# vshiv18/khoice

Measured on AMD Instinct MI355X. Metric: distinct k-mers/sec (k=31, canonical), higher is better.
Workload: dtype u64

## Files before the change

khoice_amd/csrc/kh_engine.cpp:

```cpp
#include <hip/hip_runtime.h>

#include <algorithm>
#include <atomic>
#include <thread>
#include <chrono>
#include <cmath>
#include <memory>
#include <cstdarg>
#include <cstdio>
#include <cstdlib>
#include <cstring>
#include <map>
#include <mutex>
#include <string>
#include <vector>

#include "../../include/khoice_hip.h"
#include "kh_engine.h"
#include "kh_launch.h"
#include "kh_skm_rec.h"

static thread_local std::string g_last_error;

int kh_fail(int code, const char* fmt, ...) {
// ... 1602 lines not shown
    static constexpr u32 spill_cap = 1u << 20, big_cap = 16384u;
#ifdef KH_STAMPS
    Tmp d_stamps;
#endif
    explicit SkmStage(kh_ctx* c) : pin{c} {}
};
static int skm_prepare(kh_ctx* c, int nseq, const uint8_t* const* seqs, const uint64_t* lens, int on_device,
                       const int* group_of, int ngroups, int k, bool by_group, u32 force_slots, u32 fan_hint, SkmStage* s) {
    TagLayout* L = &s->L;
    if (!skm_form_k(k)) return KH_OK;
    if ((!by_group && nseq > KH_TAG_MAX_OPS) || ngroups > KH_TAG_MAX_OPS) return KH_OK;
    KHCHK(tag_layout(L, nseq, group_of, ngroups, by_group));
    if (L->nbins > (u32)KH_TAG_MAX_BINS) return KH_OK;
    const u64 positions = kmer_positions(nseq, lens, k, &s->bases);
    if (!skm_plan(k, positions, std::max(L->fan, fan_hint), force_slots, c->cus, &s->g)) return KH_OK;
    const SkmGeometry& g = s->g;
    const size_t rec_bytes = g.two ? 32 : 16;
    const size_t reg1_bytes = rec_bytes * (size_t)g.nb1 * g.cap1, reg2_bytes = rec_bytes * (size_t)g.nslots * g.cap2;
    HIPCHK(hipSetDevice(c->dev));
    {
        size_t free_b = 0, total_b = 0;
        if (hipMemGetInfo(&free_b, &total_b) == hipSuccess &&
            reg1_bytes + reg2_bytes + s->bases + (64u << 20) > free_b + c->pool.cached_bytes)
            return KH_OK;
    }
    hipStream_t st = c->st;

    u32 tile_pos = KH_TILE;
    {
        const u64 want_tiles = 8ull * (u64)std::max(1, c->cus);
        while (tile_pos > (u32)KH_SUBTILE && (positions + tile_pos - 1) / tile_pos < want_tiles) tile_pos >>= 1;
    }
    std::vector<KhSeg> segs(nseq);
    std::vector<u64> pack_off(nseq);
    std::vector<KhTile> tiles;
    u64 seq_bytes = 0;
    for (int i = 0; i < nseq; ++i) {
        KhSeg& sg = segs[i];
        memset(&sg, 0, sizeof sg);
        const u64 len = lens[L->perm[i]];
        pack_off[i] = seq_bytes;
        sg.len = len;
        sg.npos = len >= (u64)k ? len - k + 1 : 0;
        sg.ntiles = (u32)((sg.npos + tile_pos - 1) / tile_pos);
        sg.tile_base = (u32)tiles.size();
        for (u32 t = 0; t < sg.ntiles; ++t) tiles.push_back(KhTile{(u32)i, t});
        seq_bytes += (len + 15) & ~15ull;
    }
    seq_bytes += 256;
    const u32 ntiles = (u32)tiles.size();
    const u32 reps = g.ugrid;
    const size_t hist_words = (size_t)reps * L->nbins;
    const size_t off_ctl = 8 * hist_words, off_inst = off_ctl + 32, off_dup = off_inst + 8 * (size_t)nseq,
                 off_cur1 = off_dup + 8 * 64, off_cur2 = off_cur1 + 4 * (size_t)KH_SKM_CUR1_STRIDE * g.nb1,
                 off_ginfo = off_cur2 + 4 * (size_t)((g.nslots + 3) & ~3u), off_tags = off_ginfo + 256,
                 off_segs = off_tags + (((size_t)nseq + 15) & ~(size_t)15), off_tiles = off_segs + sizeof(KhSeg) * nseq,
                 ws_bytes = off_tiles + sizeof(KhTile) * (size_t)std::max<u32>(1, ntiles);
    const u32 spill_cap = SkmStage::spill_cap;
    bool need_pack = false;
    for (int i = 0; i < nseq; ++i)
        if (!(on_device && (reinterpret_cast<uintptr_t>(seqs[L->perm[i]]) & 15) == 0)) need_pack = true;
    TMP_ALLOC(s->d_seq, c, need_pack ? seq_bytes : 256);
    TMP_ALLOC(s->d_ws, c, ws_bytes);
    TMP_ALLOC(s->d_reg1, c, reg1_bytes);
    TMP_ALLOC(s->d_reg2, c, reg2_bytes);
    TMP_ALLOC(s->d_spill, c, (size_t)spill_cap * (rec_bytes + 4) + (size_t)SkmStage::big_cap * 4);
    const size_t up_bytes = ws_bytes - off_ginfo;
    const size_t down_bytes = off_cur1;
    PIN_ALLOC(s->pin, up_bytes + down_bytes + 64);
    u8* h_up = static_cast<u8*>(s->pin.p);
    s->h_down = h_up + ((up_bytes + 63) & ~(size_t)63);
    c->prof_begin(KC_COPY_IN);
    for (int i = 0; i < nseq; ++i) {
        const uint8_t* src = seqs[L->perm[i]];
        if (on_device && (reinterpret_cast<uintptr_t>(src) & 15) == 0) { segs[i].seq = src; continue; }
        segs[i].seq = s->d_seq.as<u8>() + pack_off[i];
        if (!segs[i].len) continue;
        HIPCHK(hipMemcpyAsync(s->d_seq.as<u8>() + pack_off[i], src, segs[i].len,
                              on_device ? hipMemcpyDeviceToDevice : hipMemcpyHostToDevice, st));
        c->stat.text_packed += segs[i].len;
    }
    memcpy(h_up + (off_segs - off_ginfo), segs.data(), sizeof(KhSeg) * nseq);
    if (ntiles) memcpy(h_up + (off_tiles - off_ginfo), tiles.data(), sizeof(KhTile) * (size_t)ntiles);
    L->words(reinterpret_cast<u32*>(h_up), h_up + (off_tags - off_ginfo), group_of);
    u8* wsp = s->d_ws.as<u8>();
    HIPCHK(hipMemsetAsync(wsp, 0, off_ginfo, st));
    HIPCHK(hipMemcpyAsync(wsp + off_ginfo, h_up, up_bytes, hipMemcpyHostToDevice, st));
    c->prof_end();

    KhSkmJob& job = s->job;
    job.seg_tag = by_group ? wsp + off_tags : nullptr;
    job.segs = reinterpret_cast<const KhSeg*>(wsp + off_segs);
    job.tiles = reinterpret_cast<const KhTile*>(wsp + off_tiles);
    job.reg1 = s->d_reg1.as<uint4>();
    job.reg2 = s->d_reg2.as<uint4>();
    job.cur1 = reinterpret_cast<u32*>(wsp + off_cur1);
    job.cur2 = reinterpret_cast<u32*>(wsp + off_cur2);
    job.inst = reinterpret_cast<unsigned long long*>(wsp + off_inst);
    job.dup = reinterpret_cast<unsigned long long*>(wsp + off_dup);
    job.ginfo = reinterpret_cast<const u32*>(wsp + off_ginfo);
    job.hist = reinterpret_cast<unsigned long long*>(wsp);
    job.ctl = reinterpret_cast<u32*>(wsp + off_ctl);
    job.tile_pos = tile_pos;
    job.k = k; job.m = g.m; job.w = g.w; job.nmax = g.nmax;
    job.nslots = g.nslots; job.S = g.S; job.nb1 = g.nb1; job.cap1 = g.cap1; job.cap2 = g.cap2;
    job.nbins = L->nbins; job.abase = L->abase; job.reps = reps; job.nops = by_group ? (u32)ngroups : (u32)nseq;
    job.spill_rec = s->d_spill.as<uint4>();
    job.spill_slot = reinterpret_cast<u32*>(s->d_spill.as<u8>() + (size_t)spill_cap * rec_bytes);
    job.big_list = reinterpret_cast<u32*>(s->d_spill.as<u8>() + (size_t)spill_cap * (rec_bytes + 4));
    job.spill_cap = spill_cap;
    job.big_cap = SkmStage::big_cap;
    s->ntiles = ntiles;
#ifdef KH_STAMPS
    const u64 nst = std::max<u64>(ntiles, g.nslots);
    TMP_ALLOC(s->d_stamps, c, 128 * nst);
    HIPCHK(hipMemsetAsync(s->d_stamps.b->p, 0, 128 * nst, st));
    kh_debug_set_stamps_skm(s->d_stamps.as<u64>());
#endif
    c->prof_begin(KC_SKM_SCATTER);
    if (g.two) kh_launch_skm2_scatter(job, ntiles, st);
    else kh_launch_skm_scatter(job, ntiles, st);
    c->prof_end();
#ifdef KH_STAMPS
    report_stamps(c, "skm_scatter (second sub-tile: codes / hashes / minima / slots+count / - / append / barrier / -)", s->d_stamps.b, ntiles);
    HIPCHK(hipMemsetAsync(s->d_stamps.b->p, 0, 128 * nst, st));
    kh_debug_set_stamps_skm(nullptr);
#endif
    c->prof_begin(KC_SKM_REGROUP);
    if (g.two) kh_launch_skm2_regroup(job, st);
    else kh_launch_skm_regroup(job, st);
    c->prof_end();
#ifdef KH_STAMPS
    kh_debug_set_stamps_skm(s->d_stamps.as<u64>());
#endif
    s->staged = true;
    return KH_OK;
}
static int exp1_skm(kh_ctx* c, const Exp1In& in, uint64_t* within_hist, uint64_t* across_hist, uint64_t* distinct_per_seq,
                    bool* done, bool by_group = false) {
    *done = false;
    SkmStage s(c);
    KHCHK(skm_prepare(c, in.nseq, in.seqs, in.lens, in.on_device, in.group_of, in.ngroups, in.k, by_group, 0, 0, &s));
    if (!s.staged) return KH_OK;
    const TagLayout& L = s.L;
    const SkmGeometry& g = s.g;
    const KhSkmJob& job = s.job;
    hipStream_t st = c->st;
    c->prof_begin(KC_SKM_UNION);
    if (g.two) kh_launch_skm2_union(job, in.cs, g.ugrid, st);
    else kh_launch_skm_union(job, in.cs, g.ugrid, st);
    c->prof_end();
    HIPCHK(hipGetLastError());
#ifdef KH_STAMPS
    report_stamps(c, "skm_union (scan barrier / owner / expand / insert / barrier / read-out / barrier / flush)", s.d_stamps.b, g.nslots);
    kh_debug_set_stamps_skm(nullptr);
#endif
    if (getenv("KHOICE_SKM_DEBUG")) {
        std::vector<u32> h1(g.nb1), h2(g.nslots);
        HIPCHK(hipMemcpy2DAsync(h1.data(), 4, job.cur1, 4 * (size_t)KH_SKM_CUR1_STRIDE, 4, g.nb1, hipMemcpyDeviceToHost, st));
        HIPCHK(hipMemcpyAsync(h2.data(), job.cur2, 4 * (size_t)g.nslots, hipMemcpyDeviceToHost, st));
        u32 hc[8];
        HIPCHK(hipMemcpyAsync(hc, job.ctl, 32, hipMemcpyDeviceToHost, st));
        HIPCHK(hipStreamSynchronize(st));
        u64 t1 = 0, t2 = 0;
        u32 m1 = 0, m2 = 0;
        for (u32 v : h1) { t1 += v; m1 = std::max(m1, v); }
        for (u32 v : h2) { t2 += v; m2 = std::max(m2, v); }
        fprintf(stderr, "[skm] k=%d m=%d w=%u nmax=%u positions=%llu records=%llu (%.2f k-mers each) nb1=%u S=%u nslots=%u | "
                        "coarse: mean %.0f max %u cap %u | slot: mean %.1f max %u cap %u | tiles %u x %u | expanded: %u k-mers | errors %u spilled %u overfull slots %u\n",
                in.k, g.m, g.w, g.nmax, (unsigned long long)g.positions, (unsigned long long)t1, (double)g.positions / std::max<u64>(1, t1),
                g.nb1, g.S, g.nslots, (double)t1 / g.nb1, m1, g.cap1, (double)t2 / g.nslots, m2, g.cap2, s.ntiles, job.tile_pos, hc[3], hc[0], hc[5], hc[6]);
    }
    u8* h_down = s.h_down;
    u8* wsp = s.d_ws.as<u8>();
    auto down = [&](const void* d) { return h_down + (static_cast<const u8*>(d) - wsp); };
    const size_t down_bytes = down(job.cur1) - h_down;
    HIPCHK(hipMemcpyAsync(h_down, wsp, down_bytes, hipMemcpyDeviceToHost, st));
    HIPCHK(hipStreamSynchronize(st));
    const u64* h_hist = reinterpret_cast<const u64*>(h_down);
    const u32* h_ctl = reinterpret_cast<const u32*>(down(job.ctl));
    if (h_ctl[6] && !(h_ctl[0] & (KH_ERR_CAPACITY | KH_ERR_ORDER))) {
        if (h_ctl[5] > SkmStage::spill_cap || h_ctl[6] > SkmStage::big_cap) { c->stat.retries++; return KH_OK; }
        c->stat.big_slots += h_ctl[6];
        c->prof_begin(KC_SKM_BIG);
        if (g.two) kh_launch_skm2_big(job, in.cs, h_ctl[6], st);
        else kh_launch_skm_big(job, in.cs, h_ctl[6], st);
        c->prof_end();
        HIPCHK(hipGetLastError());
        HIPCHK(hipMemcpyAsync(h_down, wsp, down_bytes, hipMemcpyDeviceToHost, st));
        HIPCHK(hipStreamSynchronize(st));
    }
    const u64* h_inst = reinterpret_cast<const u64*>(down(job.inst));
    const u64* h_dup = reinterpret_cast<const u64*>(down(job.dup));
    if (h_ctl[0] & (KH_ERR_CAPACITY | KH_ERR_ORDER)) {
        c->stat.retries++;
        return KH_OK;
    }
    c->stat.skm_records += h_ctl[2];
    if (!L.by_group) {
        c->stat.bases += s.bases;
        c->stat.builds += L.nseq;
        u64 inst = 0, dsum = 0;
        for (int i = 0; i < L.nseq; ++i) {
            const u64 d = h_inst[i] - h_dup[i];
            inst += h_inst[i];
            dsum += d;
            if (distinct_per_seq) distinct_per_seq[L.perm[i]] = d;
        }
        c->stat.kmers += inst;
        c->stat.distinct += dsum;
        c->stat.setop_in += dsum;
    }
    c->stat.setops++;
    std::vector<u64> bins(L.nbins, 0);
    L.add_bins(bins, h_hist, job.reps);
    L.fold(c, bins, within_hist, across_hist, in.hist_len);
    *done = true;
    return KH_OK;
}
static bool bmp_form_k(int k) {
    int max_k = KH_BMP_MAX_K;
    if (const char* e = getenv("KHOICE_BMP_MAX_K")) max_k = std::min(KH_BMP_INST_MAX_K, atoi(e));
    return !(k > max_k || getenv("KHOICE_NO_BMP") || getenv("KHOICE_NO_SKM") || skm_form_k(k));
}
struct BmpStage {
    u64 nwords = 0, nsplits = 0, bases = 0;
    u32 range_bits = 0, nranges = 0, tile_pos = 0;
    u32 rwaves = 0, rgrid = 0;
    std::vector<KhBmpSplit> splits;
    std::vector<KhBmpOp> ops;
    std::vector<u64> pack_off;
    u64 seq_bytes = 0;
    bool need_pack = false;
};
static int bmp_plan(kh_ctx* c, int k, int nops, const uint8_t* const* seqs, const uint64_t* lens, int on_device,
                    u64 extra_rows, BmpStage* s, bool* fits) {
    *fits = false;
    const u64 nwords = k >= 3 ? 1ull << (2 * k - 6) : 1;
    u32 range_bits = KH_BMP_RANGE_BITS;
    if (const char* e = getenv("KHOICE_BMP_RANGE_BITS")) range_bits = (u32)std::min(20, std::max(16, atoi(e)));
    range_bits = std::min<u32>(range_bits, (u32)std::max(6, 2 * k));
    const u32 nranges = (u32)((nwords * 64) >> range_bits);
    u32 tile_pos = KH_BMP_TILE;
    if (const char* e = getenv("KHOICE_BMP_TILE_POS"))
        tile_pos = std::min<u32>(KH_BMP_TILE, std::max<u32>(16, (u32)strtoul(e, nullptr, 10) & ~15u));
    u64 bases = 0, maxpos = 0;
    const u64 positions = kmer_positions(nops, lens, k, &bases);
    for (int i = 0; i < nops; ++i) maxpos = std::max<u64>(maxpos, lens[i] >= (u64)k ? lens[i] - k + 1 : 0);
    const u64 want_wgs = 4ull * (u64)std::max(1, c->cus);
    const u64 want_splits = std::max<u64>(1, want_wgs / nranges);
    u64 split_pos = std::max<u64>((positions + want_splits - 1) / want_splits, std::max<u64>(tile_pos, (1ull << range_bits) / 16));
    if (const char* e = getenv("KHOICE_BMP_SPLIT_POS")) split_pos = std::max<u64>(16, strtoull(e, nullptr, 10));
    split_pos = (split_pos + 15) & ~15ull;
    auto count_splits = [&](u64 sp) {
        u64 n = 0;
        for (int i = 0; i < nops; ++i) {
            const u64 npos = lens[i] >= (u64)k ? lens[i] - k + 1 : 0;
            n += std::max<u64>(1, (npos + sp - 1) / sp);
        }
        return n;
    };
    HIPCHK(hipSetDevice(c->dev));
    u64 budget = 1ull << 30;
    {
        size_t free_b = 0, total_b = 0;
        if (hipMemGetInfo(&free_b, &total_b) == hipSuccess) budget = (free_b + c->pool.cached_bytes) / 4;
    }
    if (const char* e = getenv("KHOICE_BMP_MAX_BYTES")) budget = strtoull(e, nullptr, 10);
    u64 nsplits = count_splits(split_pos);
    while ((nsplits + extra_rows) * nwords * 8 > budget && split_pos < maxpos) {
        split_pos *= 2;
        nsplits = count_splits(split_pos);
    }
    if ((nsplits + extra_rows) * nwords * 8 > budget || nsplits * nranges > 0x7fffffffull) return KH_OK;
    const size_t lds_build = kh_bmp_build_lds_bytes(range_bits, tile_pos);
    if (lds_build > 160u * 1024u) return KH_OK;
    if (getenv("KHOICE_BMP_DEBUG"))
        fprintf(stderr, "[bmp] k=%d range_bits=%u R=%u tile_pos=%u split_pos=%llu splits=%llu workgroups=%llu bitmap_bytes=%llu\n", k,
                range_bits, nranges, tile_pos, (unsigned long long)split_pos, (unsigned long long)nsplits,
                (unsigned long long)(nsplits * nranges), (unsigned long long)((nsplits + extra_rows) * nwords * 8));

    s->nwords = nwords; s->nsplits = nsplits; s->bases = bases;
    s->range_bits = range_bits; s->nranges = nranges; s->tile_pos = tile_pos;
    s->ops.resize(nops);
    s->pack_off.resize(nops);
    s->splits.reserve(nsplits);
    for (int i = 0; i < nops; ++i) {
        const u64 len = lens[i], npos = len >= (u64)k ? len - k + 1 : 0;
        s->pack_off[i] = s->seq_bytes;
        s->seq_bytes += (len + 15) & ~15ull;
        if (!(on_device && (reinterpret_cast<uintptr_t>(seqs[i]) & 15) == 0)) s->need_pack = true;
        s->ops[i].split0 = (u32)s->splits.size();
        u64 p0 = 0;
        do {
            const u64 p1 = std::min(npos, p0 + split_pos);
            s->splits.push_back(KhBmpSplit{nullptr, len, p0, p1, (u32)i, 0});
            p0 = p1;
        } while (p0 < npos);
        s->ops[i].nsplits = (u32)s->splits.size() - s->ops[i].split0;
    }
    s->seq_bytes += 256;
    const u64 rblocks = (nwords + 63) / 64;
    s->rwaves = rblocks <= 256 ? 16u : 4u;
    s->rgrid = (u32)std::min<u64>(rblocks, 8ull * (u64)std::max(1, c->cus));
    *fits = true;
    return KH_OK;
}
// ... 1737 lines not shown
```

khoice_amd/csrc/kh_skm.hip:

```cpp
#include <hip/hip_runtime.h>

#include "kh_device.h"
#include "kh_launch.h"

#ifdef KH_STAMPS
__device__ u64* g_skm_stamps = nullptr;
void kh_debug_set_stamps_skm(u64* p) { (void)hipMemcpyToSymbol(HIP_SYMBOL(g_skm_stamps), &p, sizeof p); }
#define SKM_STAMP(idx)                                                                     \
    do {                                                                                   \
        __builtin_amdgcn_sched_barrier(0);                                                 \
        if (threadIdx.x == 0 && g_skm_stamps)                                              \
            g_skm_stamps[((u64)blockIdx.y * gridDim.x + blockIdx.x) * 16 + (idx)] = __builtin_amdgcn_s_memtime(); \
        __builtin_amdgcn_sched_barrier(0);                                                 \
    } while (0)
#else
#define SKM_STAMP(idx) do {} while (0)
#endif

#ifdef KH_MARKS
#define SKM_MARK(name) asm volatile("; ===== MARK " name ::: "memory")
#else
#define SKM_MARK(name) do {} while (0)
#endif
#ifndef KH_TUNE_SKM_SCATTER_PREFETCH
// ... 106 lines not shown
            bm |= bm >> ((u32)k - cover);
            vm = ~(u32)bm;
        }
        u32 cont = 0;
#pragma unroll
        for (int j = 1; j < (int)SKM_PPT; ++j)
            if (cur[j] == cur[j - 1]) cont |= 1u << j;
        cont &= vm & (vm << 1);
        const u32 tr = (vm >> 31) ? 1u + (u32)__builtin_clz(~cont | 1u) : 0u;
        const u32 lead = 1u + (u32)__builtin_ctz(~(cont >> 1));
        const u32 p_min = (u32)__builtin_amdgcn_update_dpp(0, (int)cur[SKM_PPT - 1], 0x138, 0xf, 0xf, false);
        const u32 p_tr = (u32)__builtin_amdgcn_update_dpp(0, (int)tr, 0x138, 0xf, 0xf, false);
        const bool merge_in = lane != 0 && p_tr != 0 && (vm & 1u) && p_min == cur[0] && p_tr + lead <= nmax;
        const u32 ext = next_lane(merge_in ? lead : 0u, 0u);
        const u32 starts = (vm & ~cont) & ~(merge_in ? 1u : 0u);
        auto run_len = [&](u32 c, u32 e, u32 s) -> u32 {
            const u32 len = 1u + (u32)__builtin_ctzll(~((u64)c >> (s + 1)));
            return s + len == SKM_PPT ? len + e : len;
        };
        lrun[tid] = make_uint2(cont, ext);
        bool split;
        {
            u32 y = cont, c = 1;
            while (2 * c <= nmax) { y &= y >> c; c <<= 1; }
            split = (y & (y >> (nmax - c))) != 0u;
        }
        const bool any_split = __ballot(split) != 0;
        u32 nrec = (u32)__popc(starts);
        if (any_split && split) {
            nrec = 0;
            u32 st = starts;
            while (st) {
                const u32 s = (u32)__builtin_ctz(st);
                st &= st - 1;
                nrec += (run_len(cont, ext, s) + nmax - 1) / nmax;
            }
        }
        {
            const u32 tot = wave_scan_add((u32)__popc(vm));
            if (lane == KH_WAVE - 1 && tot) atomicAdd(&misc[1], tot);
        }
        if (stamp) SKM_STAMP(3);
        if (stamp) SKM_STAMP(4);
        uint2* const dsc = reinterpret_cast<uint2*>(L.stage);
        bool done = false, first_round = true;
        while (true) {
            const u32 mine = done ? 0u : nrec;
            const u32 incl = wave_scan_add(mine);
            if (lane == KH_WAVE - 1) misc[4 + wid] = incl;
            __syncthreads();
            u32 excl = incl - mine, total = 0;
            for (u32 q = 0; q < SKM_NT / 64; ++q) {
                const u32 v = misc[4 + q];
                excl += q < wid ? v : 0u;
                total += v;
            }
            if (first_round) { tile_recs += total; first_round = false; }
            const bool fits = staged + excl + mine <= SKM_CAP;
            const bool wrote = !done && fits;
            if (stamp) SKM_STAMP(9);
            if (wrote) {
                const u32 at = staged + excl;
                if (!split) {
                    u32 sv = starts, tb = tid << 5;
                    asm volatile("" : "+v"(sv), "+v"(tb));
#pragma unroll
                    for (int j = 0; j < (int)SKM_PPT; ++j)
                        if (sv & (1u << j))
                            dsc[2 * (at + (u32)__popc(sv & ((1u << j) - 1u)))] = make_uint2(tb | (u32)j, cur[j]);
                } else {
                    u32 sl[SKM_PPT];
#pragma unroll
                    for (int j = 0; j < (int)SKM_PPT; ++j) sl[j] = cur[j];
                    u32 a = at, st = starts;
                    while (st) {
                        const u32 s = (u32)__builtin_ctz(st);
                        st &= st - 1;
                        const u32 minv = pick32(sl, s);
                        for (u32 s2 = s, len = run_len(cont, ext, s); len; ) {
                            const u32 n = len < nmax ? len : nmax;
                            dsc[2 * a++] = make_uint2((n << 16) | (tid << 5) | s2, minv);
                            s2 += n;
                            len -= n;
                        }
                    }
                }
            }
            const u64 wm = __ballot(wrote);
            if (wm) {
                const u32 base = staged + (u32)__builtin_amdgcn_readlane((int)excl, 0);
                const u32 cnt = (u32)__builtin_amdgcn_readlane((int)incl, 63 - __builtin_clzll(wm));
                __builtin_amdgcn_fence(__ATOMIC_RELEASE, "workgroup");
                __builtin_amdgcn_wave_barrier();
                __builtin_amdgcn_fence(__ATOMIC_ACQUIRE, "workgroup");
                for (u32 r = lane; r < cnt; r += KH_WAVE) {
                    const u32 at = base + r;
                    const uint2 d = dsc[2 * at];
                    const u32 src = (d.x >> 5) & (SKM_NT - 1), s = d.x & 31u;
                    const uint2 li = lrun[src];
                    const u32 n = (d.x >> 16) ? (d.x >> 16) : run_len(li.x, li.y, s);
                    const u32 slot = slot_of(d.y, nslots);
                    const u32 coarse = (u32)(((u64)slot * smagic) >> 40), fine = slot - coarse * S;
                    const u32 bp = src * SKM_PPT + s, sh = 2 * (bp & 15u);
                    const u32* cq = code + (bp >> 4);
                    const u32 c0 = cq[0], c1 = cq[1], c2 = cq[2], c3 = cq[3], c4 = cq[4];
                    const int bits = 2 * ((int)n + k - 1);
                    auto keep = [](u32 x, int b) -> u32 { return b >= 32 ? x : (b <= 0 ? 0u : x & ((1u << b) - 1u)); };
                    const u32 x0 = __builtin_amdgcn_alignbit(c1, c0, sh);
                    const u32 x1 = keep(__builtin_amdgcn_alignbit(c2, c1, sh), bits - 32);
                    const u32 x2 = keep(__builtin_amdgcn_alignbit(c3, c2, sh), bits - 64);
                    const u32 x3 = keep(__builtin_amdgcn_alignbit(c4, c3, sh), bits - 96) | SkmRec1::header(fine, rtag, n);
                    L.stage[at] = make_uint4(x0, x1, x2, x3);
                    L.sid[at] = (u16)coarse;
                    atomicAdd(&L.bcnt[coarse], 1u);
                }
            }
            if (wrote) done = true;
            if (stamp) SKM_STAMP(5);
            const u32 room = SKM_CAP - staged;
            if (total <= room) {
                staged += total;
                if (stamp) SKM_STAMP(6);
                __syncthreads();
                if (stamp) { SKM_STAMP(7); SKM_STAMP(8); }
                break;
            }
            if (tid == 0) misc[2] = 0;
            __syncthreads();
            if (fits && mine) atomicMax(&misc[2], excl + mine);
            __syncthreads();
            const u32 part = misc[2];
            if (stamp) SKM_STAMP(10);
            skm_flush<SKM_NT, SKM_CAP, false>(L, staged + part, jb.nb1, jb.cur1, jb.reg1, jb.cap1, jb.ctl);
            if (stamp) SKM_STAMP(11);
            staged = 0;
        }
    }
    __syncthreads();
    if (staged) skm_flush<SKM_NT, SKM_CAP, false>(L, staged, jb.nb1, jb.cur1, jb.reg1, jb.cap1, jb.ctl);
    if (tid == 0 && misc[1]) atomicAdd(&jb.inst[t.seg], (unsigned long long)misc[1]);
    if (tid == 0 && tile_recs) atomicAdd(jb.ctl + 2, tile_recs);
}

#ifndef KH_TUNE_SKM_UE
#define KH_TUNE_SKM_UE 2
#endif
constexpr u32 SKM_UE = KH_TUNE_SKM_UE;
constexpr u32 SKM_OB = SKM_UE == 2 ? 4 : 3;
constexpr u32 SKM_PASSES = SKM_UE == 2 ? 3 : 2;
template <u32 NT, u32 T> struct SkmUnionGeo {
    static constexpr u32 T2 = 128;
    static constexpr u32 MAXREC = NT;
    static constexpr u32 MAXCH = SKM_PASSES * NT;
    static constexpr size_t LDS = (size_t)T * 16 + (size_t)T2 * 16 + 1024 + 128 + 256 + (size_t)SKM_HSTRIPE_WORDS * 4 +
                                  (size_t)MAXCH * 2 + (size_t)MAXREC * 4;
    static_assert(MAXREC * 16 <= T * 4, "records are staged in the first half of the key plane");
    static_assert(T2 <= NT && T % 4 == 0, "table planes are cleared 16 bytes at a time");
    static_assert((T & (T - 1u)) == 0u, "table indices wrap by a mask");
};
using SkmUnion = SkmUnionGeo<1024, 4096>;
u32 kh_skm_union_max_cap2() { return SkmUnion::MAXREC; }
u32 kh_skm_union_per_cu() { return 2u; }
size_t kh_skm_union_lds_bytes() { return SkmUnion::LDS; }

__device__ __forceinline__ u32 key_hash2(u32 lo, u32 hi) { return (lo ^ hi) * 0x9E3779B1u; }

struct Skm1Consts {
    u32 kml, kmh;
    u32 fsh;
    u32 tsh;
    u32 tsh_sub;
    bool tsh_high;
    __device__ __forceinline__ explicit Skm1Consts(const int k)
        : kml((u32)kh_mask(2 * k)), kmh((u32)(kh_mask(2 * k) >> 32)), fsh(64u - 2u * (u32)k), tsh(2u * (u32)k - 2u),
          tsh_sub(tsh >= 32u ? tsh - 32u : tsh), tsh_high(tsh >= 32u) {}
};
template <int E, class F>
__device__ __forceinline__ void skm1_expand(const uint4 r0, const u32 first, const Skm1Consts& kc, F&& f) {
    const u64 clo = ((u64)r0.y << 32) | r0.x, chi = ((u64)r0.w << 32) | r0.z;
    const u32 sh = 2u * first;
    const u64 lo = sh ? (clo >> sh) | (chi << (64u - sh)) : clo, hi = chi >> sh;
    const u32 xl = (u32)lo & kc.kml, xh = (u32)(lo >> 32) & kc.kmh;
    const u64 fw = kh_revpairs64(((u64)xh << 32) | xl) >> kc.fsh;
    u32 fl = (u32)fw, fh = (u32)(fw >> 32), rl = ~xl & kc.kml, rh = ~xh & kc.kmh;
    const u32 t = (u32)((lo >> kc.tsh) | (hi << (64u - kc.tsh)));
    const u32 tc = ~t;
#pragma unroll
    for (int e = 0; e < E; ++e) {
        if (e) {
            fh = __builtin_amdgcn_alignbit(fh, fl, 30) & kc.kmh;
            fl = ((fl << 2) | ((t >> (2 * e)) & 3u)) & kc.kml;
            rl = __builtin_amdgcn_alignbit(rh, rl, 2);
            rh >>= 2;
            if (kc.tsh_high) rh |= ((tc >> (2 * e)) & 3u) << kc.tsh_sub; else rl |= ((tc >> (2 * e)) & 3u) << kc.tsh_sub;
        }
        const bool fwd = fh < rh || (fh == rh && fl < rl);
        f((u32)e, fwd ? fl : rl, fwd ? fh : rh);
    }
}
struct SkmClaim1 {
    unsigned long long* tkey;
    u32 okey_off;
    unsigned long long empty, K;
    __device__ __forceinline__ u32 operator()(const bool second, const u32 S) const {
        const unsigned long long o2 = atomicCAS(tkey + (second ? okey_off : 0u) + S, empty, K);
        return o2 == empty ? SKM_FRESH : (o2 == K ? SKM_SAME_KEY : SKM_OTHER_KEY);
    }
};

#ifdef KH_STAMPS
#define SKM_USTAMP(idx)                                                                    \
    do {                                                                                   \
        __builtin_amdgcn_sched_barrier(0);                                                 \
        if (threadIdx.x == 0 && g_skm_stamps) g_skm_stamps[(u64)slot * 16 + (idx)] = __builtin_amdgcn_s_memtime(); \
        __builtin_amdgcn_sched_barrier(0);                                                 \
    } while (0)
#else
#define SKM_USTAMP(idx) do {} while (0)
#endif

template <u32 NT, u32 T>
__global__ __launch_bounds__(NT, 8) void k_skm_union(const KhSkmJob jb, u32 cs) {
    extern __shared__ __attribute__((aligned(16))) u8 lds_raw[];
    using G = SkmUnionGeo<NT, T>;
    constexpr u32 T2 = G::T2, NW = NT / 64;
    constexpr u32 T2SH = 25;
    constexpr int E = (int)SKM_UE;
    constexpr u64 EMPTY = ~0ull;
    u8* p = lds_raw;
    unsigned long long* tkey = reinterpret_cast<unsigned long long*>(p);   p += (size_t)T * 8;
    u32* tmlo = reinterpret_cast<u32*>(p);                                 p += (size_t)T * 4;
    u32* tmhi = reinterpret_cast<u32*>(p);                                 p += (size_t)T * 4;
    unsigned long long* okey = reinterpret_cast<unsigned long long*>(p);   p += (size_t)T2 * 8;
    u32* omlo = reinterpret_cast<u32*>(p);                                 p += (size_t)T2 * 4;
    u32* omhi = reinterpret_cast<u32*>(p);                                 p += (size_t)T2 * 4;
    uint4* gtab = reinterpret_cast<uint4*>(p);                             p += 1024;
    u32* scratch = reinterpret_cast<u32*>(p);                              p += 128;
    u32* dupc = reinterpret_cast<u32*>(p);                                 p += 256;
    u32* hstripe = reinterpret_cast<u32*>(p);                              p += (size_t)SKM_HSTRIPE_WORDS * 4;
    u16* owner = reinterpret_cast<u16*>(p);                                p += (size_t)G::MAXCH * 2;
    u32* rmask = reinterpret_cast<u32*>(p);
    uint4* stage = reinterpret_cast<uint4*>(tkey);
    u32* dd = reinterpret_cast<u32*>(tkey) + T;
    const u32 tid0 = threadIdx.x, wid = __builtin_amdgcn_readfirstlane(tid0 >> 6);
    u32 tid = tid0, lane = lane_id();
    const u32 nbins = jb.nbins, cap2 = jb.cap2, nslots = jb.nslots, stride = gridDim.x;
    const int k = jb.k;
    const u32 sshift = nbins <= 72u ? 2u : (nbins <= 144u ? 1u : 0u), smask = (1u << sshift) - 1u;
    auto clear_keys = [&]() {
        uint4* k4 = reinterpret_cast<uint4*>(tkey);
        for (u32 i = tid; i < T / 2; i += NT) k4[i] = make_uint4(0xffffffffu, 0xffffffffu, 0xffffffffu, 0xffffffffu);
    };
#if !(defined(KH_ABLATE) && KH_ABLATE == 3)
    constexpr bool MASKS_SELF_CLEAN = true;
#else
    constexpr bool MASKS_SELF_CLEAN = false;
#endif
    auto zero_masks = [&]() {
        for (u32 i = tid; i < T / 2; i += NT) reinterpret_cast<uint4*>(tmlo)[i] = make_uint4(0u, 0u, 0u, 0u);
        if (tid < T2) { omlo[tid] = 0u; omhi[tid] = 0u; }
    };
    auto clear_masks = [&]() {
        if (!MASKS_SELF_CLEAN) zero_masks();
        unsigned long long e0 = EMPTY;
        asm volatile("" : "+v"(e0));
        if (tid < T2) okey[tid] = e0;
    };
    typedef const u32 __attribute__((address_space(4))) * ConstU32;
    const ConstU32 counts = (ConstU32)(unsigned long long)jb.cur2;
    const u32 fit = cap2 < G::MAXREC ? cap2 : G::MAXREC;
    auto count_of = [&](u32 sl) -> u32 {
        const u32 n = sl < nslots ? counts[sl] : 0u;
        return n <= fit ? n : 0u;
    };
    SKM_MARK("init");
    if (MASKS_SELF_CLEAN) zero_masks();
    if (tid < (u32)KH_TAG_MAX_OPS) {
        const u32 g = jb.ginfo[tid], g0 = g & 0xffu, gn = (g >> 8) & 0xffu;
        const u64 gm = gn ? (gn >= 64u ? ~0ull : ((1ull << gn) - 1ull)) << g0 : 0ull;
        gtab[tid] = make_uint4((u32)gm, (u32)(gm >> 32), (g >> 16) << sshift, 0u);
        dupc[tid] = 0;
    }
    if (tid < SKM_HSTRIPE_WORDS) hstripe[tid] = 0;
    if (tid == 0) scratch[0] = 0;
    const u32 kml = (u32)kh_mask(2 * k), kmh = (u32)(kh_mask(2 * k) >> 32);
    const u32 fsh = 64u - 2u * (u32)k;
    const u32 tsh = 2u * (u32)k - 2u;
    const bool tsh_high = tsh >= 32u;
    const u32 tsh_sub = tsh_high ? tsh - 32u : tsh;
    auto eval_mask = [&](u32 mlo, u32 mhi) -> bool {
        const u32 lsel = lane & smask;
        u32 ng = 0;
        do {
            const u32 first = mlo ? (u32)__builtin_ctz(mlo) : 32u + (u32)__builtin_ctz(mhi);
            const uint4 g = gtab[first];
            u32 c = (u32)__popc(mlo & g.x) + (u32)__popc(mhi & g.y);
            c = c < cs ? c : cs;
            atomicAdd(&hstripe[g.z + (c << sshift) + lsel], 1u);
            const u32 keep_hi = mlo ? ~0u : mhi - 1u;
            mlo &= ~g.x & (mlo - 1u);
            mhi &= ~g.y & keep_hi;
            ++ng;
        } while (mlo | mhi);
        if (ng == 1u) return true;
        atomicAdd(&hstripe[((jb.abase + (ng < cs ? ng : cs)) << sshift) + lsel], 1u);
        return false;
    };
    u32 st_full = 0, st_exp = 0;
    u32 slot = blockIdx.x;
    u32 nrec = count_of(slot);
    u32 nrec_next = count_of(slot + stride);
    uint4 rr = tid < nrec ? (jb.reg2 + (u64)slot * cap2)[tid] : make_uint4(0, 0, 0, 0);
    for (; slot < nslots; slot += stride) {
        tid = tid0;
        asm volatile("" : "+v"(tid));
        lane = tid & (KH_WAVE - 1u);
        const uint4* __restrict__ reg = jb.reg2 + (u64)slot * cap2;
        const u32 nrec_after = count_of(slot + 2u * stride);
        if (!nrec && counts[slot] > fit) {
            if (tid0 == 0) {
                const u32 at = atomicAdd(jb.ctl + 6, 1u);
                if (at < jb.big_cap) jb.big_list[at] = slot;
            }
        }
        u32 nj = 0;
        const u32 tg = SkmRec1::tag(rr.w);
        const u32 rx = rr.x, ry = rr.y, rz = rr.z, rw = rr.w;
        {
            u32 z = 0;
            asm volatile("" : "+v"(z));
            for (u32 i = tid; i < T / 4; i += NT) reinterpret_cast<uint4*>(dd)[i] = make_uint4(z, z, z, z);
        }
        if (tid < nrec) {
            nj = SkmRec1::n(rr.w);
            stage[tid] = rr;
            rmask[tid] = 1u << (tg & 31u);
        }
        SKM_USTAMP(0);
        __syncthreads();
        SKM_USTAMP(1);
        SKM_MARK("dedup");
        if (__builtin_amdgcn_ballot_w64(nj != 0)) {
            u32 h = rx * 0x9E3779B1u ^ ry * 0x85EBCA77u ^ rz * 0xC2B2AE3Du ^ SkmRec1::content_hash_word(rw) * 0x27D4EB2Fu;
            h ^= h >> 15;
            h *= 0x2C1B3C6Du;
            u32 hp = (u32)(((u64)h * T) >> 32);
            const u32 nch = (nj + (u32)E - 1u) / (u32)E;
            bool pend = nj != 0, won = false;
            while (__builtin_amdgcn_ballot_w64(pend)) {
                if (pend) {
                    const u32 old = atomicCAS(&dd[hp], 0u, tid + 1u);
                    if (old == 0u) {
                        won = true;
                        pend = false;
                    } else {
                        const uint4 o = stage[old - 1u];
                        if (o.x == rx && o.y == ry && o.z == rz && SkmRec1::same_content(o.w, rw)) {
                            const u32 bit = 1u << (tg & 31u);
                            const u32 was = atomicOr(&rmask[old - 1u], bit);
                            if (was & bit) {
                                atomicAdd(&dupc[tg], nj);
                                rmask[tid] = 0u;
                            }
                            pend = false;
                        } else {
                            hp = (hp + 1u) & (T - 1u);
                        }
                    }
                }
            }
            const u32 mine = won ? (nch | (nj << 16)) : 0u;
            const u32 incl = wave_scan_add(mine);
            u32 wbase = 0;
            if (lane == KH_WAVE - 1 && incl) wbase = atomicAdd(&scratch[0], incl);
            wbase = (u32)__builtin_amdgcn_readlane((int)wbase, KH_WAVE - 1);
            if (won) {
                const u32 cstart = (wbase + incl - mine) & 0xffffu;
                if (cstart + nch <= G::MAXCH) {
#pragma unroll
                    for (u32 cc = 0; cc < (1u << SKM_OB); ++cc)
                        if (cc < nch) owner[cstart + cc] = (u16)((tid << SKM_OB) | cc);
                }
            }
        }
        SKM_MARK("dedup_end");
        SKM_USTAMP(2);
        __syncthreads();
        const u32 sc0 = scratch[0];
        if ((sc0 & 0xffffu) > G::MAXCH) {
            if (tid < nrec && rmask[tid] == 0u) {
                const u32 w = stage[tid].w;
                atomicSub(&dupc[SkmRec1::tag(w)], SkmRec1::n(w));
            }
            __syncthreads();
        }
        rr = tid < nrec_next ? (jb.reg2 + (u64)(slot + stride) * cap2)[tid] : make_uint4(0, 0, 0, 0);
        clear_keys();
        clear_masks();
        u32 C = sc0 & 0xffffu, N = sc0 >> 16;
        SKM_USTAMP(3);
        SKM_MARK("after_scan");
        st_full = N > st_full ? N : st_full;
        st_exp += N;
        if (C > G::MAXCH) {
            if (tid == 0) {
                if (jb.big_list) {
                    const u32 at = atomicAdd(jb.ctl + 6, 1u);
                    if (at < jb.big_cap) jb.big_list[at] = slot;
                } else atomicOr(jb.ctl, KH_ERR_CAPACITY);
            }
            C = 0;
            N = 0;
        }
#if defined(KH_ABLATE) && KH_ABLATE == 1
        C = 0; N = 0;
#endif
        __syncthreads();
        if (tid == 0) scratch[0] = 0;
        SKM_MARK("owner_done");
        SKM_USTAMP(4);
        const u32 R = (N + T - 1) / T;
        const u32 ctid = tid;
        for (u32 q = 0; q < R; ++q) {
            if (q) { clear_keys(); clear_masks(); __syncthreads(); }
            unsigned long long emptyv = EMPTY;
            asm volatile("" : "+v"(emptyv));
            u32 made[SKM_PASSES][E / 2];
#pragma unroll
            for (u32 ps = 0; ps < SKM_PASSES; ++ps)
#pragma unroll
                for (int e = 0; e < E / 2; ++e) made[ps][e] = 0u;
            u32 ones = 0;
#pragma unroll
            for (u32 pass = 0; pass < SKM_PASSES; ++pass) {
                if (pass * NT >= C) break;
                const u32 c = pass * NT + ctid;
                u64 kreg[E];
                u32 slot_[E], act = 0, bits = 0, half = 0;
#pragma unroll
                for (int e = 0; e < E; ++e) { kreg[e] = EMPTY; slot_[e] = 0; }
                if (c < C) {
                    const u32 o = owner[c], ri = o >> SKM_OB, first = (o & ((1u << SKM_OB) - 1u)) * (u32)E;
                    const uint4 r0 = reg[ri];
                    bits = rmask[ri];
                    half = SkmRec1::half(r0.w);
                    const u32 left = SkmRec1::n(r0.w) - first;
                    const u32 cnt = left < (u32)E ? left : (u32)E;
                    const u64 clo = ((u64)r0.y << 32) | r0.x, chi = ((u64)r0.w << 32) | r0.z;
                    const u32 sh = 2u * first;
                    const u64 lo = sh ? (clo >> sh) | (chi << (64u - sh)) : clo, hi = chi >> sh;
                    const u32 xl = (u32)lo & kml, xh = (u32)(lo >> 32) & kmh;
                    const u64 fw = kh_revpairs64(((u64)xh << 32) | xl) >> fsh;
                    u32 fl = (u32)fw, fh = (u32)(fw >> 32), rl = ~xl & kml, rh = ~xh & kmh;
                    const u32 t = (u32)((lo >> tsh) | (hi << (64u - tsh)));
                    const u32 tc = ~t;
#pragma unroll
                    for (int e = 0; e < E; ++e) {
                        if (e) {
                            fh = __builtin_amdgcn_alignbit(fh, fl, 30) & kmh;
                            fl = ((fl << 2) | ((t >> (2 * e)) & 3u)) & kml;
                            rl = __builtin_amdgcn_alignbit(rh, rl, 2);
                            rh >>= 2;
                            if (tsh_high) rh |= ((tc >> (2 * e)) & 3u) << tsh_sub; else rl |= ((tc >> (2 * e)) & 3u) << tsh_sub;
                        }
                        const bool fwd = fh < rh || (fh == rh && fl < rl);
                        const u32 cl = fwd ? fl : rl, ch = fwd ? fh : rh;
                        const u32 h = key_hash2(cl, ch);
                        kreg[e] = ((u64)ch << 32) | cl;
                        slot_[e] = (u32)(((u64)h * T) >> 32);
                        if (R != 1 && (u32)e < cnt && (((h >> 4) & 0xffffu) * R) >> 16 == q) act |= 1u << e;
                    }
                    if (R == 1) act = (1u << cnt) - 1u;
                }
#if defined(KH_ABLATE) && KH_ABLATE == 2
                if (kreg[0] != 0x1234567ull) act = 0;
#endif
                SKM_MARK("expanded");
                if (!__builtin_amdgcn_ballot_w64(act != 0)) continue;
                u32* const mp = half ? tmhi : tmlo;
                u32 was[E];
#pragma unroll
                for (int e = 0; e < E; ++e) was[e] = 0u;
                u32 mk = 0;
                for (u32 round = 0; round < (u32)KH_TUNE_SKM_FULL_ROUNDS && __builtin_amdgcn_ballot_w64(act != 0); ++round) {
                    unsigned long long old[E];
#pragma unroll
                    for (int e = 0; e < E; ++e)
                        old[e] = (act & (1u << e)) ? atomicCAS(&tkey[slot_[e]], emptyv, (unsigned long long)kreg[e]) : 0ull;
#pragma unroll
                    for (int e = 0; e < E; ++e) {
                        if (act & (1u << e)) {
                            const bool fresh = old[e] == emptyv;
                            if (fresh || old[e] == kreg[e]) {
                                was[e] = atomicOr(mp + slot_[e], bits);
                                act &= ~(1u << e);
                                if (fresh) mk |= 1u << e;
                            } else {
                                slot_[e] = (slot_[e] + 1u) & (T - 1u);
                            }
                        }
                    }
                }
                SKM_USTAMP(9);
                SKM_MARK("rounds_done");
                u32 f16[E];
#pragma unroll
                for (int e = 0; e < E; ++e) f16[e] = (mk >> e) & 1u ? (0x8000u | slot_[e]) : 0u;
                while (__builtin_amdgcn_ballot_w64(act != 0)) {
                    const bool have_one = act != 0;
                    const u32 es = have_one ? (u32)__builtin_ctz(act) : 0u;
                    u64 K = 0;
#pragma unroll
                    for (int e = 0; e < E; ++e)
                        if (es == (u32)e) K = kreg[e];
                    const u32 H = key_hash2((u32)K, (u32)(K >> 32));
                    u32 S = ((H ^ (H >> 15)) * 0x85EBCA77u) >> T2SH, probes = 0, level = 1;
                    bool mine = have_one;
                    u32 where = 0;
                    while (__builtin_amdgcn_ballot_w64(mine)) {
                        if (mine) {
                            unsigned long long* kp = level == 1 ? okey : tkey;
                            const unsigned long long o2 = atomicCAS(&kp[S], emptyv, (unsigned long long)K);
                            if (o2 == emptyv || o2 == K) {
                                u32* mp2 = level == 1 ? (half ? omhi : omlo) : mp;
                                u32 d = atomicOr(mp2 + S, bits) & bits;
                                while (d) { atomicAdd(&dupc[half * 32u + (u32)__builtin_ctz(d)], 1u); d &= d - 1u; }
                                if (o2 == emptyv) where = 0x8000u | (level == 1 ? 0x4000u : 0u) | S;
                                mine = false;
                            } else {
                                ++probes;
                                if (level == 1 && probes >= 8u) {
                                    level = 2; probes = 0;
                                    S = (u32)(((u64)H * T) >> 32) + (u32)KH_TUNE_SKM_FULL_ROUNDS;
                                    S = S & (T - 1u);
                                } else if (level == 2 && probes >= T) {
                                    atomicOr(jb.ctl, KH_ERR_CAPACITY);
                                    mine = false;
                                } else {
                                    S = level == 1 ? ((S + 1u) & (T2 - 1u)) : ((S + 1u) & (T - 1u));
                                }
                            }
                        }
                    }
                    if (have_one) {
                        act &= ~(1u << es);
#pragma unroll
                        for (int e = 0; e < E; ++e)
                            if (es == (u32)e) f16[e] = where;
                    }
                }
                SKM_MARK("serial_done");
#pragma unroll
                for (int e = 0; e < E / 2; ++e) made[pass][e] = f16[2 * e] | (f16[2 * e + 1] << 16);
                {
                    u32 d = 0;
#pragma unroll
                    for (int e = 0; e < E; ++e) d |= was[e] & bits;
                    if (d) {
#pragma unroll
                        for (int e = 0; e < E; ++e) {
                            u32 de = was[e] & bits;
                            while (de) { atomicAdd(&dupc[half * 32u + (u32)__builtin_ctz(de)], 1u); de &= de - 1u; }
                        }
                    }
                }
            }
            SKM_MARK("insert_done");
            SKM_USTAMP(5);
            __syncthreads();
            SKM_USTAMP(6);
#pragma unroll
            for (u32 pass = 0; pass < SKM_PASSES; ++pass) {
                u32 any = 0;
#pragma unroll
                for (int e = 0; e < E / 2; ++e) any |= made[pass][e];
#if defined(KH_ABLATE) && KH_ABLATE == 3
                if (any != 0x7654321u) any = 0;
#endif
                if (!__builtin_amdgcn_ballot_w64(any != 0)) continue;
#pragma unroll
                for (int e = 0; e < E; ++e) {
                    const u32 f = (made[pass][e >> 1] >> (16 * (e & 1))) & 0xffffu;
                    if (f & 0x8000u) {
                        const u32 at = f & 0x3fffu;
                        const bool second = f & 0x4000u;
                        u32 mlo, mhi;
                        if (MASKS_SELF_CLEAN) {
                            mlo = atomicExch((second ? omlo : tmlo) + at, 0u);
                            mhi = atomicExch((second ? omhi : tmhi) + at, 0u);
                        } else {
                            mlo = (second ? omlo : tmlo)[at];
                            mhi = (second ? omhi : tmhi)[at];
                        }
                        if (eval_mask(mlo, mhi)) ++ones;
                    }
                }
            }
            if (__builtin_amdgcn_ballot_w64(ones != 0)) {
                ones = wave_scan_add(ones);
                if (lane == KH_WAVE - 1) atomicAdd(&hstripe[(jb.abase + 1u) << sshift], ones);
            }
            SKM_MARK("readout_done");
            SKM_USTAMP(7);
            if (q + 1 < R) __syncthreads();
        }
        SKM_USTAMP(8);
        nrec = nrec_next;
        nrec_next = nrec_after;
    }
    __syncthreads();
    tid = tid0;
    lane = tid & (KH_WAVE - 1u);
    unsigned long long* __restrict__ rep = jb.hist + (u64)(blockIdx.x % jb.reps) * nbins;
    for (u32 i = tid; i < nbins; i += NT) {
        u32 v = 0;
        for (u32 j = 0; j <= smask; ++j) v += hstripe[(i << sshift) + j];
        if (v) atomicAdd(&rep[i], (unsigned long long)v);
    }
    if (tid < (u32)KH_TAG_MAX_OPS && dupc[tid]) atomicAdd(&jb.dup[tid], (unsigned long long)dupc[tid]);
    if (tid == 0) {
        if (st_full > T) atomicMax(jb.ctl + 1, st_full);
        atomicAdd(jb.ctl + 3, st_exp);
    }
}

constexpr u32 SKM_BIG_T = 4096, SKM_BIG_T2 = 128;
struct SkmBig1 {
    using Rec = SkmRec1;
    using Consts = Skm1Consts;
    using Key = unsigned long long;
    static constexpr u32 T = SKM_BIG_T, T2 = SKM_BIG_T2, KEY_BYTES = 8, BATCH = 256, OB = SKM_OB;
    static constexpr int E = (int)SKM_UE;
    template <class F> static __device__ __forceinline__ void expand(const SkmRecord<1>& r, const u32 first, const Consts& kc, F&& f) {
        skm1_expand<E>(r.v[0], first, kc, [&](const u32 e, const u32 cl, const u32 ch) __attribute__((always_inline)) { f(e, ((u64)ch << 32) | cl); });
    }
    static __device__ __forceinline__ u32 hash(const Key K) { return key_hash2((u32)K, (u32)(K >> 32)); }
    static __device__ __forceinline__ SkmClaim1 claim(u8* kmain, const u32 okey_off, const Key K) {
        return SkmClaim1{reinterpret_cast<unsigned long long*>(kmain), okey_off, ~0ull, K};
    }
};

static size_t skm_pack_lds_bytes(u32 nt) { return (size_t)nt * 16 + (size_t)nt * 4 * 4 + (size_t)nt * 4 + 64; }

template <u32 NT>
__global__ __launch_bounds__(NT) void k_skm_pack(const KhSkmPackJob jb) {
    extern __shared__ __attribute__((aligned(16))) u8 lds_raw[];
    constexpr u32 T = 4 * NT, TSH = NT == 1024 ? 20u : (NT == 512 ? 21u : 22u);
    static_assert(NT == 1024 || NT == 512 || NT == 256, "table of 4 NT entries, a power of two");
    uint4* stage = reinterpret_cast<uint4*>(lds_raw);
    u32* dd = reinterpret_cast<u32*>(lds_raw + (size_t)NT * 16);
    u32* rmask = dd + T;
    u32* scratch = rmask + NT;
    const u32 tid = threadIdx.x, lane = lane_id();
    const u32 slot = blockIdx.x;
    u32 nrec = jb.cur2[slot];
    nrec = nrec < jb.cap2 ? nrec : jb.cap2;
    if (nrec > NT) {
        if (tid == 0) atomicOr(jb.ctl, KH_ERR_CAPACITY);
        nrec = NT;
    }
    const uint4 rr = tid < nrec ? (jb.reg2 + (u64)slot * jb.cap2)[tid] : make_uint4(0, 0, 0, 0);
    reinterpret_cast<uint4*>(dd)[tid] = make_uint4(0u, 0u, 0u, 0u);
    if (tid == 0) { scratch[0] = 0; scratch[1] = 0; }
    const u32 tg = SkmRec1::tag(rr.w);
    u32 nj = 0;
    if (tid < nrec) {
        nj = SkmRec1::n(rr.w);
        stage[tid] = rr;
        rmask[tid] = 1u << (tg & 31u);
        if (tg >= 32u) atomicOr(jb.ctl, KH_ERR_ORDER);
    }
    __syncthreads();
    bool won = false;
    if (__builtin_amdgcn_ballot_w64(nj != 0)) {
        u32 h = rr.x * 0x9E3779B1u ^ rr.y * 0x85EBCA77u ^ rr.z * 0xC2B2AE3Du ^ SkmRec1::content_hash_word(rr.w) * 0x27D4EB2Fu;
        h ^= h >> 15;
        h *= 0x2C1B3C6Du;
        u32 hp = h >> TSH;
        bool pend = nj != 0;
        while (__builtin_amdgcn_ballot_w64(pend)) {
            if (pend) {
                const u32 old = atomicCAS(&dd[hp], 0u, tid + 1u);
                if (old == 0u) { won = true; pend = false; }
                else {
                    const uint4 o = stage[old - 1u];
                    if (o.x == rr.x && o.y == rr.y && o.z == rr.z && SkmRec1::same_content(o.w, rr.w)) {
                        const u32 bit = 1u << (tg & 31u);
                        const u32 was = atomicOr(&rmask[old - 1u], bit);
                        if ((was & bit) && jb.dup) atomicAdd(&jb.dup[tg & 31u], (unsigned long long)nj);
                        pend = false;
                    } else hp = (hp + 1u) & (T - 1u);
                }
            }
        }
    }
    const u32 incl = wave_scan_add(won ? 1u : 0u);
    u32 wbase = 0;
    if (lane == KH_WAVE - 1 && incl) wbase = atomicAdd(&scratch[0], incl);
    wbase = (u32)__builtin_amdgcn_readlane((int)wbase, KH_WAVE - 1);
    __syncthreads();
    const u32 nsurv = scratch[0];
    const u32 part = slot / jb.spp;
    if (tid == 0) {
        const u32 sub = slot % jb.nsub;
        const u64 subcap = jb.part_cap / jb.nsub;
        u32 base = nsurv ? atomicAdd(&jb.part_cursor[part * jb.nsub + sub], nsurv) : 0u;
        if ((u64)base + nsurv > subcap) { atomicOr(jb.ctl, KH_ERR_CAPACITY); base = 0; scratch[0] = 0; }
        base += (u32)(sub * subcap);
        scratch[1] = base;
        jb.slot_count[slot] = nsurv;
        jb.slot_off[slot] = base;
    }
    __syncthreads();
    if (won && scratch[0]) {
        const u64 at = (u64)scratch[1] + wbase + incl - 1u;
        if (at < jb.part_cap) {
            jb.out_rec[(u64)part * jb.part_cap + at] = rr;
            jb.out_mask[(u64)part * jb.part_cap + at] = rmask[tid];
        }
    }
}

// ... 353 lines not shown
```

Baseline: 109.6 billion.

## Move dedup hash table to dedicated LDS and defer table clears off critical path

The record-dedup hash table gets its own small LDS region sized to the record count, instead of sharing the key plane. Entries now store hash bits alongside the record index, so most mismatches are rejected without reading the staged record. Records are compared in place, and each winner clears its own slot after the barrier, which removes the per-slot full-table clear. Key and mask clears move to after the insert barrier of the last round, removing one barrier from the common path. In exchange, the owner table shrinks and overflowing chunks take an extra two-barrier fallback, and the reuse of LDS regions becomes more complex.

```diff
diff --git a/khoice_amd/csrc/kh_engine.cpp b/khoice_amd/csrc/kh_engine.cpp
--- a/khoice_amd/csrc/kh_engine.cpp
+++ b/khoice_amd/csrc/kh_engine.cpp
@@ -1778,7 +1778,7 @@
     c->prof_end();
     HIPCHK(hipGetLastError());
 #ifdef KH_STAMPS
-    report_stamps(c, "skm_union (scan barrier / owner / expand / insert / barrier / read-out / barrier / flush)", s.d_stamps.b, g.nslots);
+    report_stamps(c, "skm_union (stamps 1-8: barrier / merge / barrier + set zeroed / expand + insert / barrier / keys cleared / read-out / to the end of the slot; 9: probe rounds of the last pass done)", s.d_stamps.b, g.nslots);
     kh_debug_set_stamps_skm(nullptr);
 #endif
     if (getenv("KHOICE_SKM_DEBUG")) {
diff --git a/khoice_amd/csrc/kh_skm.hip b/khoice_amd/csrc/kh_skm.hip
--- a/khoice_amd/csrc/kh_skm.hip
+++ b/khoice_amd/csrc/kh_skm.hip
@@ -282,10 +282,16 @@
     static constexpr u32 T2 = 128;
     static constexpr u32 MAXREC = NT;
     static constexpr u32 MAXCH = SKM_PASSES * NT;
+    static constexpr u32 DD = MAXREC;
+    static constexpr u32 DDOVER = 1280;
+    static constexpr u32 DDCH = MAXCH - DDOVER;
     static constexpr size_t LDS = (size_t)T * 16 + (size_t)T2 * 16 + 1024 + 128 + 256 + (size_t)SKM_HSTRIPE_WORDS * 4 +
-                                  (size_t)MAXCH * 2 + (size_t)MAXREC * 4;
-    static_assert(MAXREC * 16 <= T * 4, "records are staged in the first half of the key plane");
-    static_assert(T2 <= NT && T % 4 == 0, "table planes are cleared 16 bytes at a time");
+                                  (size_t)MAXREC * 4 + (size_t)DDCH * 2 + (size_t)DD * 4;
+    static_assert(LDS <= 81920, "two workgroups per CU");
+    static_assert(DD >= MAXREC && (DD & (DD - 1u)) == 0u && DD <= (1u << 11),
+                  "every record finds an entry; indices wrap by a mask; record number + 1 takes 11 bits");
+    static_assert(DDOVER * 2 <= DD * 4 && (DDCH * 2) % 16 == 0 && (DDOVER * 2) % 16 == 0, "the chunk table's tail is cleared 16 bytes at a time");
+    static_assert(T2 <= NT && DD <= NT && T % 4 == 0, "table planes are cleared 16 bytes at a time");
     static_assert((T & (T - 1u)) == 0u, "table indices wrap by a mask");
 };
 using SkmUnion = SkmUnionGeo<1024, 4096>;
@@ -368,10 +374,10 @@
     u32* scratch = reinterpret_cast<u32*>(p);                              p += 128;
     u32* dupc = reinterpret_cast<u32*>(p);                                 p += 256;
     u32* hstripe = reinterpret_cast<u32*>(p);                              p += (size_t)SKM_HSTRIPE_WORDS * 4;
-    u16* owner = reinterpret_cast<u16*>(p);                                p += (size_t)G::MAXCH * 2;
-    u32* rmask = reinterpret_cast<u32*>(p);
-    uint4* stage = reinterpret_cast<uint4*>(tkey);
-    u32* dd = reinterpret_cast<u32*>(tkey) + T;
+    u32* rmask = reinterpret_cast<u32*>(p);                                p += (size_t)G::MAXREC * 4;
+    u16* owner = reinterpret_cast<u16*>(p);                                p += (size_t)G::DDCH * 2;
+    u32* dd = reinterpret_cast<u32*>(p);
+    constexpr u32 DDREC = 11, DDMASK = G::DD - 1u;
     const u32 tid0 = threadIdx.x, wid = __builtin_amdgcn_readfirstlane(tid0 >> 6);
     u32 tid = tid0, lane = lane_id();
     const u32 nbins = jb.nbins, cap2 = jb.cap2, nslots = jb.nslots, stride = gridDim.x;
@@ -405,6 +411,9 @@
     };
     SKM_MARK("init");
     if (MASKS_SELF_CLEAN) zero_masks();
+    clear_keys();
+    clear_masks();
+    if (tid < G::DD) dd[tid] = 0u;
     if (tid < (u32)KH_TAG_MAX_OPS) {
         const u32 g = jb.ginfo[tid], g0 = g & 0xffu, gn = (g >> 8) & 0xffu;
         const u64 gm = gn ? (gn >= 64u ? ~0ull : ((1ull << gn) - 1ull)) << g0 : 0ull;
@@ -456,45 +465,46 @@
         u32 nj = 0;
         const u32 tg = SkmRec1::tag(rr.w);
         const u32 rx = rr.x, ry = rr.y, rz = rr.z, rw = rr.w;
-        {
-            u32 z = 0;
-            asm volatile("" : "+v"(z));
-            for (u32 i = tid; i < T / 4; i += NT) reinterpret_cast<uint4*>(dd)[i] = make_uint4(z, z, z, z);
-        }
         if (tid < nrec) {
             nj = SkmRec1::n(rr.w);
-            stage[tid] = rr;
             rmask[tid] = 1u << (tg & 31u);
         }
         SKM_USTAMP(0);
         __syncthreads();
         SKM_USTAMP(1);
         SKM_MARK("dedup");
+        u32 myhp = ~0u;
+        u32 late = ~0u;
         if (__builtin_amdgcn_ballot_w64(nj != 0)) {
             u32 h = rx * 0x9E3779B1u ^ ry * 0x85EBCA77u ^ rz * 0xC2B2AE3Du ^ SkmRec1::content_hash_word(rw) * 0x27D4EB2Fu;
             h ^= h >> 15;
             h *= 0x2C1B3C6Du;
-            u32 hp = (u32)(((u64)h * T) >> 32);
+            u32 hp = (u32)(((u64)h * G::DD) >> 32);
+            const u32 ent = (h << DDREC) | (tid + 1u);
             const u32 nch = (nj + (u32)E - 1u) / (u32)E;
             bool pend = nj != 0, won = false;
             while (__builtin_amdgcn_ballot_w64(pend)) {
                 if (pend) {
-                    const u32 old = atomicCAS(&dd[hp], 0u, tid + 1u);
+                    const u32 old = atomicCAS(&dd[hp], 0u, ent);
                     if (old == 0u) {
                         won = true;
+                        myhp = hp;
                         pend = false;
+                    } else if ((old ^ ent) >> DDREC) {
+                        hp = (hp + 1u) & DDMASK;
                     } else {
-                        const uint4 o = stage[old - 1u];
+                        const u32 ro = (old & ((1u << DDREC) - 1u)) - 1u;
+                        const uint4 o = reg[ro];
                         if (o.x == rx && o.y == ry && o.z == rz && SkmRec1::same_content(o.w, rw)) {
                             const u32 bit = 1u << (tg & 31u);
-                            const u32 was = atomicOr(&rmask[old - 1u], bit);
+                            const u32 was = atomicOr(&rmask[ro], bit);
                             if (was & bit) {
                                 atomicAdd(&dupc[tg], nj);
                                 rmask[tid] = 0u;
                             }
                             pend = false;
                         } else {
-                            hp = (hp + 1u) & (T - 1u);
+                            hp = (hp + 1u) & DDMASK;
                         }
                     }
                 }
@@ -506,10 +516,12 @@
             wbase = (u32)__builtin_amdgcn_readlane((int)wbase, KH_WAVE - 1);
             if (won) {
                 const u32 cstart = (wbase + incl - mine) & 0xffffu;
-                if (cstart + nch <= G::MAXCH) {
+                if (cstart + nch <= G::DDCH) {
 #pragma unroll
                     for (u32 cc = 0; cc < (1u << SKM_OB); ++cc)
                         if (cc < nch) owner[cstart + cc] = (u16)((tid << SKM_OB) | cc);
+                } else {
+                    late = cstart;
                 }
             }
         }
@@ -517,16 +529,20 @@
         SKM_USTAMP(2);
         __syncthreads();
         const u32 sc0 = scratch[0];
+        if (myhp != ~0u) dd[myhp] = 0u;
         if ((sc0 & 0xffffu) > G::MAXCH) {
-            if (tid < nrec && rmask[tid] == 0u) {
-                const u32 w = stage[tid].w;
-                atomicSub(&dupc[SkmRec1::tag(w)], SkmRec1::n(w));
-            }
+            if (tid < nrec && rmask[tid] == 0u) atomicSub(&dupc[tg], nj);
+        } else if ((sc0 & 0xffffu) > G::DDCH) {
             __syncthreads();
+            if (late != ~0u) {
+                const u32 nch = (nj + (u32)E - 1u) / (u32)E;
+#pragma unroll
+                for (u32 cc = 0; cc < (1u << SKM_OB); ++cc)
+                    if (cc < nch) owner[late + cc] = (u16)((tid << SKM_OB) | cc);
+            }
+            __syncthreads();
         }
         rr = tid < nrec_next ? (jb.reg2 + (u64)(slot + stride) * cap2)[tid] : make_uint4(0, 0, 0, 0);
-        clear_keys();
-        clear_masks();
         u32 C = sc0 & 0xffffu, N = sc0 >> 16;
         SKM_USTAMP(3);
         SKM_MARK("after_scan");
@@ -545,10 +561,16 @@
 #if defined(KH_ABLATE) && KH_ABLATE == 1
         C = 0; N = 0;
 #endif
-        __syncthreads();
-        if (tid == 0) scratch[0] = 0;
+        const bool tail_used = (sc0 & 0xffffu) > G::DDCH && (sc0 & 0xffffu) <= G::MAXCH;
+        auto zero_tail = [&]() {
+            if (tid < G::DDOVER * 2u / 16u) reinterpret_cast<uint4*>(dd)[tid] = make_uint4(0u, 0u, 0u, 0u);
+        };
+        if (N == 0 && sc0 != 0u) {
+            __syncthreads();
+            if (tid == 0) scratch[0] = 0;
+            if (tail_used) zero_tail();
+        }
         SKM_MARK("owner_done");
-        SKM_USTAMP(4);
         const u32 R = (N + T - 1) / T;
         const u32 ctid = tid;
         for (u32 q = 0; q < R; ++q) {
@@ -696,8 +718,15 @@
                 }
             }
             SKM_MARK("insert_done");
+            SKM_USTAMP(4);
+            __syncthreads();
             SKM_USTAMP(5);
-            __syncthreads();
+            if (q + 1 == R) {
+                clear_keys();
+                clear_masks();
+                if (tid == 0) scratch[0] = 0;
+                if (tail_used) zero_tail();
+            }
             SKM_USTAMP(6);
 #pragma unroll
             for (u32 pass = 0; pass < SKM_PASSES; ++pass) {
```

Result: slower. 101.7 billion (-7.2%).
